# apache/tez

Hardware: NVIDIA B200
Metric: sorted KV GB/s (16B key / 64B val) (higher is better)
Workload: dtype u8

## Files before the change

tez_b200/csrc/emit_pipe.cuh:

```cuda
#pragma once
#include "emit_fast.cuh"

#ifndef TEZGPU_EMIT4_MIN_CTAS
#define TEZGPU_EMIT4_MIN_CTAS 3
#endif
#ifndef TEZGPU_EMIT4_MAP16
#define TEZGPU_EMIT4_MAP16 0
#endif

namespace tezgpu {

constexpr int FE4_BATCH = FE_THREADS / 32;
constexpr int FE4_UNROLL = TEZGPU_EMIT4_MAP16 ? 6 : 5;

static inline bool emit4_fits(uint32_t recs, uint32_t cpr) {
#if TEZGPU_EMIT4_MAP16
  const uint32_t rph = 16u / cpr;
  return cpr <= 8 && 16ull * ((recs + rph - 1) / rph) <= (uint64_t)FE4_UNROLL * FE_THREADS;
#else
  return cpr <= 8 && (uint64_t)recs * cpr <= (uint64_t)FE4_UNROLL * FE_THREADS;
#endif
}

struct FoldMeta {
  uint4 tail;
  uint32_t tile;
  uint32_t start;
  uint32_t end;
  uint32_t tiny;
};

__device__ __forceinline__ uint4 lds_v4(uint32_t a) {
  uint4 v;
  asm volatile("ld.shared.v4.b32 {%0,%1,%2,%3}, [%4];" : "=r"(v.x), "=r"(v.y), "=r"(v.z), "=r"(v.w) : "r"(a));
  return v;
}

template <int SUBS>
struct Emit4Smem {
  static constexpr int BATCH = SUBS > 1 ? 4 : FE4_BATCH;
  static constexpr size_t WTAB = SUBS > 1 ? (size_t)4 * 256 * 32 * 4 : 0;
  static constexpr size_t SHARED = WTAB + 256 * 4 + 4 * 256 * 4;
  static constexpr size_t GROUP = FE_IMG_BYTES + 3 * FE_MAX_RECS * 4 + (size_t)BATCH * FE_THREADS * 4 + (size_t)BATCH * sizeof(FoldMeta);
  static constexpr size_t TOTAL = SHARED + SUBS * GROUP;
};

template <int UNROLL, int SUBS>
__global__ void __launch_bounds__(FE_THREADS * SUBS, SUBS > 1 ? 1 : TEZGPU_EMIT4_MIN_CTAS) k_emit_fast4(FastEmitParams fp) {
  using L = Emit4Smem<SUBS>;
  constexpr int BATCH = L::BATCH;
  extern __shared__ __align__(16) uint8_t smem4[];
  uint32_t *s_wtab = reinterpret_cast<uint32_t *>(smem4);
  uint32_t *s_tab = reinterpret_cast<uint32_t *>(smem4 + L::WTAB);
  uint32_t *s_adv128 = s_tab + 256;
  const int sub = threadIdx.x / FE_THREADS, tid = threadIdx.x % FE_THREADS, lane = tid & 31, warp = tid >> 5;
  uint8_t *gbase = smem4 + L::SHARED + (size_t)sub * L::GROUP;
  uint8_t *s_img = gbase;
  uint32_t(*s_idx)[FE_MAX_RECS] = reinterpret_cast<uint32_t(*)[FE_MAX_RECS]>(gbase + FE_IMG_BYTES);
  uint32_t(*s_part)[FE_THREADS] = reinterpret_cast<uint32_t(*)[FE_THREADS]>(gbase + FE_IMG_BYTES + 3 * FE_MAX_RECS * 4);
  FoldMeta *s_meta = reinterpret_cast<FoldMeta *>(gbase + FE_IMG_BYTES + 3 * FE_MAX_RECS * 4 + (size_t)BATCH * FE_THREADS * 4);
  auto group_sync = [&]() {
    if (SUBS == 1) __syncthreads();
    else asm volatile("bar.sync %0, %1;" ::"r"(sub + 1), "r"(FE_THREADS) : "memory");
  };

  const EmitParams &e = fp.e;
  const uint32_t G = gridDim.x * SUBS, ntiles = fp.ntiles;
  uint32_t tile = blockIdx.x * SUBS + sub;
  if (SUBS > 1)
    for (int i = threadIdx.x; i < 4 * 256 * 32; i += FE_THREADS * SUBS) s_wtab[i] = (&e.crc->slice[0][0])[i >> 5];
  for (int i = threadIdx.x; i < 256; i += FE_THREADS * SUBS) s_tab[i] = e.crc->slice[0][i];
  for (int i = threadIdx.x; i < 4 * 256; i += FE_THREADS * SUBS) s_adv128[i] = (&e.crc->adv128[0][0])[i];
  __syncthreads();
  if (tile >= ntiles) return;
  CrcChunkFoldT<false> cf;
  cf.init(e.crc, lane);
  const uint32_t lane_pow = SUBS == 1 ? cf.lane_pow : e.crc->pow_word[4 * (31 - lane)];
  const WarpLinearMap &m_word = cf.w, &m_skip = cf.s;
  const uint32_t *wt = s_wtab + lane;
  auto next_word = [&](uint32_t x) -> uint32_t {
    if (SUBS == 1) return m_word.apply(x);
    return wt[(768u + (x & 0xFFu)) << 5] ^ wt[(512u + ((x >> 8) & 0xFFu)) << 5] ^ wt[(256u + ((x >> 16) & 0xFFu)) << 5] ^ wt[(x >> 24) << 5];
  };
  const uint32_t img_base = (uint32_t)__cvta_generic_to_shared(s_img);
  const uint8_t *__restrict__ kv = e.rec.kv;
  const uint32_t rec_size = e.rec_size, hdr_len = e.fixed_hdr_len, stride = fp.stride, cpr = fp.cpr;
  const TileDesc *__restrict__ tiles = fp.tiles;

#if TEZGPU_EMIT4_MAP16
  const uint32_t rph = 16u / cpr;
  const uint32_t hl = tid & 15u, rl = hl / cpr, pc = hl - rl * cpr;
  const bool lane_used = rl < rph;
  auto piece = [&](int u, uint32_t nr, uint32_t &j, uint32_t &c) -> bool {
    const uint32_t jp = (((uint32_t)tid >> 4) + 16u * (uint32_t)u) * rph + rl;
    c = pc;
    const uint32_t half_up = (nr + 1) >> 1;
    j = jp < half_up ? 2u * jp : 2u * (jp - half_up) + 1u;
    return lane_used && jp < nr;
  };
#else
  auto piece = [&](int u, uint32_t nr, uint32_t &j, uint32_t &c) -> bool {
    const uint32_t q = tid + u * FE_THREADS;
    const uint32_t jp = cpr == 1 ? q : __umulhi(q, fp.cpr_magic);
    c = q - jp * cpr;
    const uint32_t half_up = (nr + 1) >> 1;
    j = jp < half_up ? 2u * jp : 2u * (jp - half_up) + 1u;
    return q < nr * cpr;
  };
#endif
  const uint32_t full_nr = e.recs_per_tile;
  uint32_t pk[UNROLL], onmask = 0;
#pragma unroll
  for (int u = 0; u < UNROLL; u++) {
    uint32_t j, c;
    const bool on = piece(u, full_nr, j, c);
    pk[u] = on ? (j | (16u * c) << 8 | (j * rec_size + hdr_len + 16u * c) << 15) : 0u;
    onmask |= on ? 1u << u : 0u;
  }
  uint4 v[UNROLL];
  auto issue_gather = [&](uint32_t nr, const uint32_t *idx) {
    const uint8_t *src[UNROLL];
    bool on[UNROLL];
    if (nr == full_nr) {
#pragma unroll
      for (int u = 0; u < UNROLL; u++) {
        on[u] = (onmask >> u) & 1u;
        src[u] = kv + (uint64_t)idx[pk[u] & 0xFFu] * stride + ((pk[u] >> 8) & 0x7Fu);
      }
    } else {
#pragma unroll
      for (int u = 0; u < UNROLL; u++) {
        uint32_t j, c;
        on[u] = piece(u, nr, j, c);
        src[u] = kv + (uint64_t)idx[on[u] ? j : 0u] * stride + 16u * c;
      }
    }
    if (UNROLL == 5) asm volatile("" : "+l"(src[0]), "+l"(src[1]), "+l"(src[2]), "+l"(src[3]), "+l"(src[UNROLL - 1]));
#pragma unroll
    for (int u = 0; u < UNROLL; u++)
      if (on[u]) v[u] = ldg_stream_v4(src[u]);
  };
  const uint32_t hdr16 = (uint32_t)e.fixed_hdr[0] | (uint32_t)e.fixed_hdr[1] << 8;

  uint32_t nr0, fl0, nr1 = 0, fl1 = 0, r0_2 = 0, nr2 = 0;
  uint64_t abs0, abs1 = 0;
  {
    const TileDesc t0 = tiles[tile];
    nr0 = t0.nr; fl0 = t0.flags; abs0 = t0.abs0;
    if ((uint32_t)tid < nr0) s_idx[0][tid] = e.order[t0.r0 + tid];
    if (tile + G < ntiles) {
      const TileDesc t1 = tiles[tile + G];
      nr1 = t1.nr; fl1 = t1.flags; abs1 = t1.abs0;
      if ((uint32_t)tid < nr1) s_idx[1][tid] = e.order[t1.r0 + tid];
    }
    if (tile + 2 * (uint64_t)G < ntiles) { r0_2 = tiles[tile + 2 * G].r0; nr2 = tiles[tile + 2 * G].nr; }
  }
  group_sync();
  issue_gather(nr0, s_idx[0]);

  uint32_t n_it = 0, slot = 0;
  for (;; tile += G, n_it++) {
    const bool has1 = tile + G < ntiles, has2 = tile + 2 * (uint64_t)G < ntiles, has3 = tile + 3 * (uint64_t)G < ntiles;
    const uint32_t nr = nr0;
    const bool first_tile = fl0 & 1u, last_tile = fl0 & 2u;
    const uint32_t lead = (uint32_t)(abs0 & 15u);
    const uint32_t rec0 = lead + (first_tile ? 4u : 0u);
    const uint32_t body_end = rec0 + nr * rec_size + (last_tile ? 2u : 0u);

    uint32_t r_idx = 0, r0_3 = 0, nr3 = 0, nr2n = 0, fl2n = 0;
    uint64_t abs2n = 0;
    if (has2) {
      if ((uint32_t)tid < nr2) r_idx = e.order[r0_2 + tid];
      const TileDesc *t2 = tiles + tile + 2 * (uint64_t)G;
      nr2n = t2->nr; fl2n = t2->flags; abs2n = t2->abs0;
    }
    if (has3) { const TileDesc *t3 = tiles + tile + 3 * (uint64_t)G; r0_3 = t3->r0; nr3 = t3->nr; }

    if (nr == full_nr) {
#pragma unroll
      for (int u = 0; u < UNROLL; u++)
        if ((onmask >> u) & 1u) sts16_unaligned(img_base + rec0 + (pk[u] >> 15), v[u]);
    } else {
#pragma unroll
      for (int u = 0; u < UNROLL; u++) {
        uint32_t j, c;
        if (piece(u, nr, j, c)) sts16_unaligned(img_base + rec0 + j * rec_size + hdr_len + 16u * c, v[u]);
      }
    }
    if ((uint32_t)tid < nr) {
      const uint32_t a = img_base + rec0 + tid * rec_size;
      if (hdr_len == 2 && !(a & 1u)) sts_b16(a, hdr16);
      else for (uint32_t b = 0; b < hdr_len; b++) sts_b8(a + b, e.fixed_hdr[b]);
    }
    if (tid == 0) {
      if (first_tile) { s_img[lead] = 'T'; s_img[lead + 1] = 'I'; s_img[lead + 2] = 'F'; s_img[lead + 3] = 0; }
      if (last_tile) { s_img[body_end - 2] = 0xFF; s_img[body_end - 1] = 0xFF; }
    }
    group_sync();

    if (has1) issue_gather(nr1, s_idx[(n_it + 1) % 3]);

    const uint32_t cb0 = rec0, cb1 = body_end;
    const uint32_t ca = cb0 >> 4, cz = cb1 >> 4;
    uint8_t *dstg = e.out + (abs0 - lead);
    uint32_t c = 0;
    if (cz > ca) {
      const uint32_t Cn = cz - ca;
      const uint32_t iters = (Cn + FE_THREADS - 1) / FE_THREADS;
      int32_t i = (int32_t)Cn + tid - (int32_t)(iters * FE_THREADS);
      uint32_t sa = img_base + 16u * (uint32_t)((int32_t)ca + i);
      uint8_t *gp = dstg + 16ll * ((int64_t)ca + i);
      for (uint32_t it = 0; it < iters; it++, i += FE_THREADS, sa += 16u * FE_THREADS, gp += 16 * FE_THREADS) {
        if (i + (31 - lane) < 0) continue;
        uint4 w = make_uint4(0, 0, 0, 0);
        if (i >= 0) {
          w = lds_v4(sa);
          if (i == 0) {
            const uint32_t b0 = 16u * ca;
            if (b0 >= lead) stg_stream_v4(gp, w);
            else for (uint32_t x = lead; x < b0 + 16u; x++) dstg[x] = s_img[x];
            const uint32_t skip = cb0 & 15u;
            if (skip) {
              uint32_t ww[4] = {w.x, w.y, w.z, w.w};
#pragma unroll
              for (uint32_t k = 0; k < 4; k++) {
                if (skip >= 4 * k + 4) ww[k] = 0;
                else if (skip > 4 * k) ww[k] &= 0xFFFFFFFFu << (8u * (skip - 4 * k));
              }
              w = make_uint4(ww[0], ww[1], ww[2], ww[3]);
            }
          } else {
            stg_stream_v4(gp, w);
          }
        }
        if (SUBS == 1) {
          c = cf.fold(c, w, it + 1 == iters);
        } else {
          uint32_t x = next_word(c ^ w.x) ^ w.y;
          x = next_word(x) ^ w.z;
          x = next_word(x) ^ w.w;
          c = (it + 1 == iters) ? next_word(x) : m_skip.apply(x);
        }
      }
    }
    s_part[slot][tid] = c;
    if (tid == 0) {
      for (uint32_t x = max(lead, 16u * cz); x < body_end; x++) dstg[x] = s_img[x];
      if (ca > (lead >> 4)) for (uint32_t x = lead; x < 16u * ca; x++) dstg[x] = s_img[x];
      FoldMeta m;
      m.tail = *reinterpret_cast<const uint4 *>(s_img + 16u * cz);
      m.tile = tile;
      m.tiny = cz > ca ? 0u : 1u;
      m.start = cz > ca ? 0u : (cb0 & 15u);
      m.end = cb1 & 15u;
      s_meta[slot] = m;
    }
    if (has2) s_idx[(n_it + 2) % 3][tid] = r_idx;
    slot++;
    group_sync();

    if (slot == (uint32_t)BATCH || !has1) {
      if ((uint32_t)warp < slot) {
        uint32_t q = 0;
#pragma unroll
        for (int k = 0; k < FE_THREADS / 32; k++) {
          q = s_adv128[q & 0xFF] ^ s_adv128[256 + ((q >> 8) & 0xFF)] ^ s_adv128[512 + ((q >> 16) & 0xFF)] ^ s_adv128[768 + (q >> 24)];
          q ^= s_part[warp][lane + 32 * k];
        }
        q = crc_multmodp(q, lane_pow);
#pragma unroll
        for (int o = 16; o > 0; o >>= 1) q ^= __shfl_xor_sync(0xffffffffu, q, o);
        if (lane == 0) {
          const FoldMeta m = s_meta[warp];
          const uint32_t tw[4] = {m.tail.x, m.tail.y, m.tail.z, m.tail.w};
          uint32_t raw = m.tiny ? 0u : q;
          for (uint32_t b = m.start; b < m.end; b++) {
            const uint32_t byte = (tw[b >> 2] >> (8u * (b & 3u))) & 0xFFu;
            raw = s_tab[(raw ^ byte) & 0xFF] ^ (raw >> 8);
          }
          const TileDesc td = tiles[m.tile];
          TileCrc tc;
          tc.raw = raw;
          tc.p = td.p;
          tc.after = td.after;
          fp.tile_crc[m.tile] = tc;
        }
      }
      slot = 0;
    }
    if (!has1) break;
    asm volatile("" : "+r"(nr2n), "+r"(fl2n), "+l"(abs2n), "+r"(r0_3), "+r"(nr3));
    nr0 = nr1; fl0 = fl1; abs0 = abs1;
    nr1 = nr2n; fl1 = fl2n; abs1 = abs2n;
    r0_2 = r0_3; nr2 = nr3;
  }
}

}
```

Baseline: 840.2.

## Stage gathered KV pieces through a cp.async shared-memory ring

After: 895.9 (median of 6 runs). +6.6%, better.

```diff
diff --git a/tez_b200/csrc/emit_pipe.cuh b/tez_b200/csrc/emit_pipe.cuh
--- a/tez_b200/csrc/emit_pipe.cuh
+++ b/tez_b200/csrc/emit_pipe.cuh
@@ -7,11 +7,16 @@
 #ifndef TEZGPU_EMIT4_MAP16
 #define TEZGPU_EMIT4_MAP16 0
 #endif
+#ifndef TEZGPU_EMIT4_STAGES
+#define TEZGPU_EMIT4_STAGES 1
+#endif
 
 namespace tezgpu {
 
 constexpr int FE4_BATCH = FE_THREADS / 32;
 constexpr int FE4_UNROLL = TEZGPU_EMIT4_MAP16 ? 6 : 5;
+constexpr size_t SM_SMEM_BYTES = 228 * 1024;
+constexpr size_t SM_SMEM_PER_CTA = 1024;
 
 static inline bool emit4_fits(uint32_t recs, uint32_t cpr) {
 #if TEZGPU_EMIT4_MAP16
@@ -38,17 +43,40 @@
 
 template <int SUBS>
 struct Emit4Smem {
-  static constexpr int BATCH = SUBS > 1 ? 4 : FE4_BATCH;
+  static constexpr int STAGES = SUBS > 1 ? 0 : TEZGPU_EMIT4_STAGES;
+  static constexpr int DEPTH = STAGES > 0 ? STAGES : 1;
+  static constexpr int NIDX = DEPTH + 1, NDESC = DEPTH + 3;
   static constexpr size_t WTAB = SUBS > 1 ? (size_t)4 * 256 * 32 * 4 : 0;
   static constexpr size_t SHARED = WTAB + 256 * 4 + 4 * 256 * 4;
-  static constexpr size_t GROUP = FE_IMG_BYTES + 3 * FE_MAX_RECS * 4 + (size_t)BATCH * FE_THREADS * 4 + (size_t)BATCH * sizeof(FoldMeta);
+  static constexpr size_t RING = FE_IMG_BYTES;
+  static constexpr size_t DESC = RING + (size_t)STAGES * FE4_UNROLL * FE_THREADS * 16;
+  static constexpr size_t META = DESC + NDESC * sizeof(TileDesc);
+  static constexpr size_t group_bytes(int batch) {
+    return META + (size_t)batch * sizeof(FoldMeta) + NIDX * FE_MAX_RECS * 4 + (size_t)batch * FE_THREADS * 4;
+  }
+  static constexpr int BATCH =
+      SUBS > 1 ? 4 : TEZGPU_EMIT4_MIN_CTAS * (SHARED + group_bytes(FE4_BATCH) + SM_SMEM_PER_CTA) <= SM_SMEM_BYTES ? FE4_BATCH : FE4_BATCH / 2;
+  static constexpr size_t IDX = META + (size_t)BATCH * sizeof(FoldMeta);
+  static constexpr size_t PART = IDX + NIDX * FE_MAX_RECS * 4;
+  static constexpr size_t GROUP = group_bytes(BATCH);
   static constexpr size_t TOTAL = SHARED + SUBS * GROUP;
 };
+static_assert(TEZGPU_EMIT4_MIN_CTAS * (Emit4Smem<1>::TOTAL + SM_SMEM_PER_CTA) <= SM_SMEM_BYTES, "k_emit_fast4 ring does not fit its CTAs/SM");
+static_assert(Emit4Smem<3>::TOTAL + SM_SMEM_PER_CTA <= SM_SMEM_BYTES, "k_emit_fast4<.,3> does not fit an SM");
+
+__device__ __forceinline__ void cp_async16(uint32_t dst, const void *src) {
+  asm volatile("cp.async.cg.shared.global [%0], [%1], 16;" ::"r"(dst), "l"(src) : "memory");
+}
+__device__ __forceinline__ void cp_async_commit() { asm volatile("cp.async.commit_group;" ::: "memory"); }
+template <int N>
+__device__ __forceinline__ void cp_async_wait() { asm volatile("cp.async.wait_group %0;" ::"n"(N) : "memory"); }
 
 template <int UNROLL, int SUBS>
 __global__ void __launch_bounds__(FE_THREADS * SUBS, SUBS > 1 ? 1 : TEZGPU_EMIT4_MIN_CTAS) k_emit_fast4(FastEmitParams fp) {
   using L = Emit4Smem<SUBS>;
-  constexpr int BATCH = L::BATCH;
+  static_assert(UNROLL <= FE4_UNROLL, "ring stage sized for FE4_UNROLL pieces per thread");
+  constexpr int BATCH = L::BATCH, D = L::DEPTH;
+  constexpr bool RING = L::STAGES > 0;
   extern __shared__ __align__(16) uint8_t smem4[];
   uint32_t *s_wtab = reinterpret_cast<uint32_t *>(smem4);
   uint32_t *s_tab = reinterpret_cast<uint32_t *>(smem4 + L::WTAB);
@@ -56,9 +84,11 @@
   const int sub = threadIdx.x / FE_THREADS, tid = threadIdx.x % FE_THREADS, lane = tid & 31, warp = tid >> 5;
   uint8_t *gbase = smem4 + L::SHARED + (size_t)sub * L::GROUP;
   uint8_t *s_img = gbase;
-  uint32_t(*s_idx)[FE_MAX_RECS] = reinterpret_cast<uint32_t(*)[FE_MAX_RECS]>(gbase + FE_IMG_BYTES);
-  uint32_t(*s_part)[FE_THREADS] = reinterpret_cast<uint32_t(*)[FE_THREADS]>(gbase + FE_IMG_BYTES + 3 * FE_MAX_RECS * 4);
-  FoldMeta *s_meta = reinterpret_cast<FoldMeta *>(gbase + FE_IMG_BYTES + 3 * FE_MAX_RECS * 4 + (size_t)BATCH * FE_THREADS * 4);
+  TileDesc *s_desc = reinterpret_cast<TileDesc *>(gbase + L::DESC);
+  FoldMeta *s_meta = reinterpret_cast<FoldMeta *>(gbase + L::META);
+  uint32_t(*s_idx)[FE_MAX_RECS] = reinterpret_cast<uint32_t(*)[FE_MAX_RECS]>(gbase + L::IDX);
+  uint32_t(*s_part)[FE_THREADS] = reinterpret_cast<uint32_t(*)[FE_THREADS]>(gbase + L::PART);
+  const uint32_t ring_base = (uint32_t)__cvta_generic_to_shared(gbase + L::RING) + 16u * tid;
   auto group_sync = [&]() {
     if (SUBS == 1) __syncthreads();
     else asm volatile("bar.sync %0, %1;" ::"r"(sub + 1), "r"(FE_THREADS) : "memory");
@@ -118,7 +148,8 @@
     onmask |= on ? 1u << u : 0u;
   }
   uint4 v[UNROLL];
-  auto issue_gather = [&](uint32_t nr, const uint32_t *idx) {
+  constexpr uint32_t STAGE_STRIDE = (uint32_t)UNROLL * FE_THREADS * 16;
+  auto issue_gather = [&](uint32_t nr, const uint32_t *idx, uint32_t stage) {
     const uint8_t *src[UNROLL];
     bool on[UNROLL];
     if (nr == full_nr) {
@@ -137,56 +168,65 @@
     }
     if (UNROLL == 5) asm volatile("" : "+l"(src[0]), "+l"(src[1]), "+l"(src[2]), "+l"(src[3]), "+l"(src[UNROLL - 1]));
 #pragma unroll
-    for (int u = 0; u < UNROLL; u++)
-      if (on[u]) v[u] = ldg_stream_v4(src[u]);
-  };
+    for (int u = 0; u < UNROLL; u++) {
+      if (!on[u]) continue;
+      if (RING) cp_async16(stage + u * FE_THREADS * 16, src[u]);
+      else v[u] = ldg_stream_v4(src[u]);
+    }
+  };
+  auto landed = [&](int u, uint32_t stage) -> uint4 { return RING ? lds_v4(stage + u * FE_THREADS * 16) : v[u]; };
   const uint32_t hdr16 = (uint32_t)e.fixed_hdr[0] | (uint32_t)e.fixed_hdr[1] << 8;
 
-  uint32_t nr0, fl0, nr1 = 0, fl1 = 0, r0_2 = 0, nr2 = 0;
-  uint64_t abs0, abs1 = 0;
-  {
-    const TileDesc t0 = tiles[tile];
-    nr0 = t0.nr; fl0 = t0.flags; abs0 = t0.abs0;
-    if ((uint32_t)tid < nr0) s_idx[0][tid] = e.order[t0.r0 + tid];
-    if (tile + G < ntiles) {
-      const TileDesc t1 = tiles[tile + G];
-      nr1 = t1.nr; fl1 = t1.flags; abs1 = t1.abs0;
-      if ((uint32_t)tid < nr1) s_idx[1][tid] = e.order[t1.r0 + tid];
-    }
-    if (tile + 2 * (uint64_t)G < ntiles) { r0_2 = tiles[tile + 2 * G].r0; nr2 = tiles[tile + 2 * G].nr; }
+  for (int k = 0; k < D + 2; k++) {
+    const uint64_t t = tile + (uint64_t)k * G;
+    if (t >= ntiles) break;
+    if (k <= D) {
+      const uint32_t r0 = tiles[t].r0, nrk = tiles[t].nr;
+      if ((uint32_t)tid < nrk) s_idx[k][tid] = e.order[r0 + tid];
+    }
+    if (tid < 8) reinterpret_cast<uint32_t *>(s_desc + k)[tid] = reinterpret_cast<const uint32_t *>(tiles + t)[tid];
   }
   group_sync();
-  issue_gather(nr0, s_idx[0]);
-
-  uint32_t n_it = 0, slot = 0;
+#pragma unroll
+  for (int k = 0; k < D; k++) {
+    if (tile + (uint64_t)k * G < ntiles) issue_gather(s_desc[k].nr, s_idx[k], ring_base + k * STAGE_STRIDE);
+    if (RING) cp_async_commit();
+  }
+
+  uint32_t n_it = 0, slot = 0, stage = ring_base;
   for (;; tile += G, n_it++) {
-    const bool has1 = tile + G < ntiles, has2 = tile + 2 * (uint64_t)G < ntiles, has3 = tile + 3 * (uint64_t)G < ntiles;
-    const uint32_t nr = nr0;
-    const bool first_tile = fl0 & 1u, last_tile = fl0 & 2u;
+    const bool has1 = tile + G < ntiles;
+    const bool hasD = tile + (uint64_t)D * G < ntiles, hasD1 = tile + (D + 1ull) * G < ntiles, hasD2 = tile + (D + 2ull) * G < ntiles;
+    const TileDesc &cur = s_desc[n_it % L::NDESC];
+    const uint32_t nr = cur.nr, fl = cur.flags;
+    const uint64_t abs0 = cur.abs0;
+    const bool first_tile = fl & 1u, last_tile = fl & 2u;
     const uint32_t lead = (uint32_t)(abs0 & 15u);
     const uint32_t rec0 = lead + (first_tile ? 4u : 0u);
     const uint32_t body_end = rec0 + nr * rec_size + (last_tile ? 2u : 0u);
 
-    uint32_t r_idx = 0, r0_3 = 0, nr3 = 0, nr2n = 0, fl2n = 0;
-    uint64_t abs2n = 0;
-    if (has2) {
-      if ((uint32_t)tid < nr2) r_idx = e.order[r0_2 + tid];
-      const TileDesc *t2 = tiles + tile + 2 * (uint64_t)G;
-      nr2n = t2->nr; fl2n = t2->flags; abs2n = t2->abs0;
-    }
-    if (has3) { const TileDesc *t3 = tiles + tile + 3 * (uint64_t)G; r0_3 = t3->r0; nr3 = t3->nr; }
-
+    uint32_t r_idx = 0, d_word = 0;
+    if (hasD1) {
+      const TileDesc &t1 = s_desc[(n_it + D + 1) % L::NDESC];
+      if ((uint32_t)tid < t1.nr) r_idx = e.order[t1.r0 + tid];
+    }
+    if (hasD2 && tid < 8) d_word = reinterpret_cast<const uint32_t *>(tiles + tile + (D + 2ull) * G)[tid];
+
+    if (RING) cp_async_wait<D - 1>();
     if (nr == full_nr) {
 #pragma unroll
       for (int u = 0; u < UNROLL; u++)
-        if ((onmask >> u) & 1u) sts16_unaligned(img_base + rec0 + (pk[u] >> 15), v[u]);
+        if ((onmask >> u) & 1u) sts16_unaligned(img_base + rec0 + (pk[u] >> 15), landed(u, stage));
     } else {
 #pragma unroll
       for (int u = 0; u < UNROLL; u++) {
         uint32_t j, c;
-        if (piece(u, nr, j, c)) sts16_unaligned(img_base + rec0 + j * rec_size + hdr_len + 16u * c, v[u]);
-      }
-    }
+        if (piece(u, nr, j, c)) sts16_unaligned(img_base + rec0 + j * rec_size + hdr_len + 16u * c, landed(u, stage));
+      }
+    }
+    if (hasD) issue_gather(s_desc[(n_it + D) % L::NDESC].nr, s_idx[(n_it + D) % L::NIDX], stage);
+    if (RING) cp_async_commit();
+    stage = (n_it + 1) % D == 0 ? ring_base : stage + STAGE_STRIDE;
     if ((uint32_t)tid < nr) {
       const uint32_t a = img_base + rec0 + tid * rec_size;
       if (hdr_len == 2 && !(a & 1u)) sts_b16(a, hdr16);
@@ -197,8 +237,6 @@
       if (last_tile) { s_img[body_end - 2] = 0xFF; s_img[body_end - 1] = 0xFF; }
     }
     group_sync();
-
-    if (has1) issue_gather(nr1, s_idx[(n_it + 1) % 3]);
 
     const uint32_t cb0 = rec0, cb1 = body_end;
     const uint32_t ca = cb0 >> 4, cz = cb1 >> 4;
@@ -255,7 +293,8 @@
       m.end = cb1 & 15u;
       s_meta[slot] = m;
     }
-    if (has2) s_idx[(n_it + 2) % 3][tid] = r_idx;
+    if (hasD1) s_idx[(n_it + D + 1) % L::NIDX][tid] = r_idx;
+    if (hasD2 && tid < 8) reinterpret_cast<uint32_t *>(s_desc + (n_it + D + 2) % L::NDESC)[tid] = d_word;
     slot++;
     group_sync();
 
@@ -289,11 +328,7 @@
       slot = 0;
     }
     if (!has1) break;
-    asm volatile("" : "+r"(nr2n), "+r"(fl2n), "+l"(abs2n), "+r"(r0_3), "+r"(nr3));
-    nr0 = nr1; fl0 = fl1; abs0 = abs1;
-    nr1 = nr2n; fl1 = fl2n; abs1 = abs2n;
-    r0_2 = r0_3; nr2 = nr3;
-  }
-}
-
-}
+  }
+}
+
+}
```
